# g1n0st/drake

Measured on AMD Instinct MI355X. Metric: mpm_substeps_per_sec_1M_particles, higher is better.
Workload: dtype f32

## Files before the change

### drake_amd/csrc/mpm_device.h

```cpp
#pragma once
#include <hip/hip_runtime.h>
#include <stdint.h>

#include "mpm_math.h"

namespace mpm {

constexpr int FREE_ZONE = 2;
constexpr int TILE_W = 4 + 2 * FREE_ZONE + 2;
constexpr int TILE_N = TILE_W * TILE_W * TILE_W;

constexpr unsigned ERR_DRIFT = 1u;
constexpr unsigned ERR_CAPACITY = 2u;
constexpr unsigned ERR_DOMAIN = 4u;
constexpr unsigned ERR_RANGE = 8u;
constexpr unsigned ERR_HALO = 16u;
constexpr unsigned ERR_SLABS = 32u;

constexpr unsigned VF_MARK = 0x7FB0A5C3u;
constexpr unsigned VF_CHUNK = 32;
__host__ __device__ inline size_t vf_entry(unsigned k, unsigned j) {
    return (size_t)(k / VF_CHUNK) * (8u * VF_CHUNK) + j * VF_CHUNK + (k % VF_CHUNK);
}
struct PSet {
    float4* q[4];
    int* pid;
    float4* fq[4];
    float* f8;
    float* c8;
};

MPM_DEV void unpack_C(const float4& q1, const float4& q2, const float4& q3, float* C) {
    C[0] = q2.x; C[1] = q2.y; C[2] = q2.z; C[3] = q2.w;
    C[4] = q3.x; C[5] = q3.y; C[6] = q3.z; C[7] = q3.w;
    C[8] = q1.w;
}

struct Ctl {
    int cur;
    int need_rebuild;
    unsigned error;
    unsigned skipped;
    int skip_this;
    unsigned watch_hit;
    unsigned n_home;
    unsigned n_active;
    unsigned n_items;
    unsigned rebuilds;
    unsigned ticket;
    int nfa, nva;
    int add_f, add_v;
    int nfa_new, nva_new;
    unsigned n_items_wanted;
    float quiet_time;
    float time_since_resort;
    float mig_quiet;
};

struct Dist {
    int on;
    int rank, world;
    int own_lo, own_hi;
    int nbr_lo, nbr_hi;
    int has_left, has_right;
    float ghost_w;
    float vert_w;
    float hyst;
    int zone_cells;
    float mig_delta;
    float mig_reach;
    unsigned* mig_min;
    unsigned char* prev;
};

MPM_DEV float dist_xi(float x, float dxinv) { return x * dxinv - .5f; }
MPM_DEV bool dist_in_my_band(const Dist& d, int bx, float xi, bool face, float extra = 0.f) {
    const float w = (face ? d.ghost_w : d.vert_w) + extra;
    return (d.has_left && bx < d.own_lo && xi >= (float)d.own_lo - w) || (d.has_right && bx >= d.own_hi && xi < (float)d.own_hi + w);
}
MPM_DEV int dist_in_neighbour_bands(const Dist& d, float xi, bool face, int old = 0) {
    const float w = face ? d.ghost_w : d.vert_w;
    const float wl = w + ((old & 1) ? d.hyst : 0.f), wr = w + ((old & 2) ? d.hyst : 0.f);
    return ((d.has_left && xi < (float)d.own_lo + wl) ? 1 : 0) | ((d.has_right && xi >= (float)d.own_hi - wr) ? 2 : 0);
}

struct DP {
    int Np, Nf, Nv;
    int NpG, NfG;
    int bits;
    int nb;
    unsigned nblocks, ncells;
    unsigned capH, capA, capI;
    unsigned capS;
    int item_groups;
    int item_groups_small;
    int item_small_below;
    int dbg;
    float dx, dxinv, Dinv;
    unsigned q_stride, f_stride;
    int gated;
    unsigned watch_base;
    int lean_resort;
    int lean_g2p;
    int fem_fast;
    float anticip;
    double fix_m, fix_p, unfix_m, unfix_p;
    Material M;
    Ctl* ctl;
    unsigned long long* dbgbuf;
    PSet set[2];
    int4* fg[2];
    int4* vg[2][2];
    float3* ta;
    float3* G3;
    float* VF;
    float* f[3];
    const int* idx_orig[3];
    const int* adj_off;
    const int* adj_fc;
    int* imap;
    uint32_t* pkey;
    uint32_t* prank;
    uint32_t* src_of;
    int* dst_of;
    unsigned* tickets;
    uint32_t* halo_hdr[2];
    int halo_cls, halo_nz, halo_zlo[2], halo_zhi[2];
    int halo_pn, halo_plo[2], halo_phi[2], halo_pshift[2];
    unsigned halo_pcap;
    uint32_t* halo_pbuf[2];
    uint32_t* halo_pcnt[2];
    int* cellcnt[2];
    int* blkcnt[2];
    int* blkstart[2];
    int* lut_home;
    int* lut_act;
    unsigned* home_bits;
    uint32_t* home_block;
    int4* home_range;
    int* home_nbr_act;
    int4* item_desc;
    uint32_t* item_order;
    int4* item_flat;
    int4* item_rng;
    uint32_t* item_pos;
    int2* home_items;
    int* act_nbr_items;
    int* home_ngroups;
    int4* home_groups;
    uint32_t* act_block;
    int* act_nbr_home;
    float4* slab;
    uint32_t* slab_mask;
    float4* gv;
    float4* gvs;
    const float4* dm_orig;
    Dist dist;
};

MPM_DEV int active_slot(const DP& p, int idx, int nf_in) { return idx < nf_in ? idx : p.Nf + (idx - nf_in); }

#ifndef MPM_DIAG
#define MPM_DIAG 0
#endif
MPM_DEV int diag_flags(const DP& p) { return MPM_DIAG ? p.dbg : 0; }

MPM_DEV void pack_F(const float* F, float4& r0, float4& r1, float& r2) {
    r0 = make_float4(F[2], F[5], F[8], F[0]);
    r1 = make_float4(F[1], F[3], F[4], F[6]);
    r2 = F[7];
}
MPM_DEV void unpack_F(const float4& r0, const float4& r1, float r2, float* F) {
    F[2] = r0.x; F[5] = r0.y; F[8] = r0.z; F[0] = r0.w;
    F[1] = r1.x; F[3] = r1.y; F[4] = r1.z; F[6] = r1.w;
    F[7] = r2;
}
// ... 41 lines not shown
```

### drake_amd/csrc/mpm_engine.hip

```cpp
#include <hip/hip_runtime.h>

#include <algorithm>
#include <chrono>
#include <cmath>
#include <cstdio>
#include <cstdlib>
#include <cstring>
#include <fstream>
#include <functional>
#include <mutex>
#include <numeric>
#include <string>
#include <thread>
#include <vector>

#include "../../include/mpm_hip.h"
#include "mpm_host.h"
#include "mpm_io.h"
#include "mpm_debug_tables.h"
#include "mpm_contact.h"
#include "mpm_chain.h"
#include "mpm_feedback.h"
#include "mpm_dist.h"
#include "mpm_cloth_host.h"
#include "mpm_bodies_host.h"
#include "mpm_dist_host.h"
#include "mpm_chain_host.h"

static std::mutex g_live_mutex;
static std::vector<mpm_engine*> g_live;

extern "C" {

const char* mpm_last_error(void) { return g_last_error.c_str(); }

int mpm_default_material(mpm_material_t* m) try {
    REQUIRE(m, "null material");
    m->youngs_modulus = 400000.f;
    m->poisson_ratio = .3f;
    m->density = 2000.f;
    m->gamma = 0.f;
    m->K = 100000.f;
    m->V = .8f;
    m->c_F = 0.f;
    m->sdf_friction = .3f;
    m->gravity = -9.8f;
    m->epsv = 1e-3f;
    m->gravity_axis = 2;
    m->wall_cells = 3;
    return 0;
} MPM_CATCH_ALL

int mpm_create(int domain_bits, const mpm_material_t* material, int device, mpm_handle_t* out) try {
    REQUIRE(out, "null handle pointer");
    REQUIRE(domain_bits >= 4 && domain_bits <= 8, "domain_bits must be in [4,8] (16^3 .. 256^3 cells)");
    int ndev = 0;
    if (hipGetDeviceCount(&ndev) != hipSuccess || ndev <= 0)
        return fail(MPM_ERR_NO_DEVICE, "no HIP device visible: the engine has no CPU fallback");
    REQUIRE(device >= 0 && device < ndev, "device ordinal out of range");
    mpm_engine* e = new mpm_engine();
    e->device = device;
    e->bits = domain_bits;
    if (material) e->mat = *material; else mpm_default_material(&e->mat);
    if (e->mat.gravity_axis < 0 || e->mat.gravity_axis > 2) {
        delete e;
        return fail(MPM_ERR_INVALID, "gravity_axis must be 0, 1 or 2");
    }
    hipError_t err = hipSetDevice(device);
    if (err == hipSuccess) err = hipStreamCreateWithFlags(&e->own_stream, hipStreamNonBlocking);
    if (err != hipSuccess) {
        delete e;
        return fail(MPM_ERR_HIP, std::string("mpm_create: ") + hipGetErrorString(err));
    }
    e->stream = e->own_stream;
    if (getenv("MPM_RESORT_EVERY")) e->check_every = std::max(1, atoi(getenv("MPM_RESORT_EVERY")));
    if (getenv("MPM_DEFER_PHASES")) e->defer_phases = atoi(getenv("MPM_DEFER_PHASES")) != 0;
    if (getenv("MPM_QUIET_FACTOR")) e->quiet_factor = std::min(1.f, std::max(0.f, (float)atof(getenv("MPM_QUIET_FACTOR"))));
    {
        std::lock_guard<std::mutex> lock(g_live_mutex);
        g_live.push_back(e);
    }
    *out = e;
    return 0;
} MPM_CATCH_ALL

static int add_cloth(mpm_engine* e, const float* pos, const float* vel, size_t n_verts, const int32_t* indices,
                     size_t n_faces, const mpm_cloth_material_t* m) {
    REQUIRE(e, "null handle");
    REQUIRE(!e->finalized, "AddQRCloth after Finalize");
    REQUIRE(pos && vel && (indices || n_faces == 0), "null input array");
    for (size_t i = 0; i < n_faces * 3; ++i)
        REQUIRE(indices[i] >= 0 && (size_t)indices[i] < n_verts, "triangle index out of range");
    REQUIRE(!(e->multi_mat || m) || e->cloths.size() < MAX_CLOTH_MATERIALS,
            "more than 256 cloths in a multi-material engine (mpm_add_qr_cloth_with_material)");
    mpm_engine::Cloth c{e->nv, n_verts, e->nf, n_faces, {}};
    c.m = m ? *m : engine_cloth_material(e);
    e->cloths.push_back(c);
    if (m) e->multi_mat = true;
    for (size_t i = 0; i < n_faces * 3; ++i) e->h_idx.push_back(indices[i] + (int)e->nv);
    e->h_pos.insert(e->h_pos.end(), pos, pos + 3 * n_verts);
    e->h_vel.insert(e->h_vel.end(), vel, vel + 3 * n_verts);
    e->nv += n_verts;
    e->nf += n_faces;
    e->np = e->nv + e->nf;
    return 0;
}

int mpm_add_qr_cloth(mpm_handle_t e, const float* pos, const float* vel, size_t n_verts, const int32_t* indices,
                     size_t n_faces) try {
    return add_cloth(e, pos, vel, n_verts, indices, n_faces, nullptr);
} MPM_CATCH_ALL

int mpm_add_qr_cloth_with_material(mpm_handle_t e, const float* pos, const float* vel, size_t n_verts,
                                   const int32_t* indices, size_t n_faces, const mpm_cloth_material_t* m) try {
    REQUIRE(e, "null handle");
    const mpm_cloth_material_t c = m ? *m : engine_cloth_material(e);
    REQUIRE(std::isfinite(c.youngs_modulus) && std::isfinite(c.poisson_ratio) && std::isfinite(c.density) &&
                std::isfinite(c.gamma) && std::isfinite(c.K) && std::isfinite(c.c_F),
            "cloth material: a field is not finite");
    REQUIRE(c.youngs_modulus > 0.f, "cloth material: youngs_modulus must be > 0");
    REQUIRE(c.poisson_ratio >= 0.f && c.poisson_ratio < .5f, "cloth material: poisson_ratio must be in [0, 0.5)");
    REQUIRE(c.density > 0.f, "cloth material: density must be > 0");
    REQUIRE(c.gamma >= 0.f && c.K >= 0.f && c.c_F >= 0.f, "cloth material: gamma, K and c_F must be >= 0");
    return add_cloth(e, pos, vel, n_verts, indices, n_faces, &c);
} MPM_CATCH_ALL

int mpm_cloth_count(mpm_handle_t e, size_t* n_out) try {
    REQUIRE(e && n_out, "null argument");
    *n_out = e->cloths.size();
    return 0;
} MPM_CATCH_ALL

int mpm_get_cloth_info(mpm_handle_t e, size_t cloth, size_t* first_vertex, size_t* n_verts, size_t* first_face,
                       size_t* n_faces, mpm_cloth_material_t* m) try {
    REQUIRE(e, "null handle");
    REQUIRE(cloth < e->cloths.size(), "cloth index out of range");
    const mpm_engine::Cloth& c = e->cloths[cloth];
    if (first_vertex) *first_vertex = c.first_vertex;
    if (n_verts) *n_verts = c.n_verts;
    if (first_face) *first_face = c.first_face;
    if (n_faces) *n_faces = c.n_faces;
    if (m) *m = c.m;
    return 0;
} MPM_CATCH_ALL

static void launch_rebuild(mpm_engine* e, DP p, bool lean, float dt) {
    if (dt > 0.f) e->last_dt = dt;
    p.anticip = e->anticipation();
    p.lean_resort = lean && !p.dist.on;
    e->checks_launched += 1;
    TraceRange tr("mpm:RebuildMapping (conditional re-sort)");
    hipLaunchKernelGGL(k_rb_count, dim3(std::min(e->g_np, e->g_rb)), dim3(256), 0, e->stream, p);
    hipLaunchKernelGGL(k_rb_tables, dim3(33), dim3(1024), 0, e->stream, p);
    hipLaunchKernelGGL(k_rb_scatter, dim3(std::min(e->g_np, e->g_rb)), dim3(256), 0, e->stream, p);
    if (e->deterministic) hipLaunchKernelGGL(k_rb_canon, dim3(512), dim3(256), 0, e->stream, p);
    hipLaunchKernelGGL(k_rb_finish, dim3((std::min(e->g_np, e->g_rb) + 7u) & ~7u), dim3(256), 0, e->stream, p);
}

static void launch_fem_faces(mpm_engine* e, const DP& p, float dt) {
    TraceRange tr("mpm:CalcFemStateAndForce (faces)");
    if (!e->nf) return;
    const dim3 g((e->g_nf + 7u) & ~7u), b(256);
    if (e->multi_mat) {
        const ClothMat* t = e->d_cloth_mat;
        if (e->fast_math) hipLaunchKernelGGL(k_fem_mat<1>, g, b, 0, e->stream, p, dt, t);
        else hipLaunchKernelGGL(k_fem_mat<0>, g, b, 0, e->stream, p, dt, t);
    } else if (e->fast_math) hipLaunchKernelGGL(k_fem<1>, g, b, 0, e->stream, p, dt);
    else hipLaunchKernelGGL(k_fem<0>, g, b, 0, e->stream, p, dt);
    if (e->damp.membrane()) hipLaunchKernelGGL(k_damp, g, b, 0, e->stream, p, e->damp.args);
}
static void launch_fem_vertices(mpm_engine* e, const DP& p, float dt) {
    TraceRange tr("mpm:CalcFemStateAndForce (vertex forces)");
    if (e->nv) hipLaunchKernelGGL(k_vforce, dim3((e->g_nv + 7u) & ~7u), dim3(256), 0, e->stream, p);
    if (e->bend.on()) hipLaunchKernelGGL(k_bend, rows_grid(e->bend.args.n_rows), dim3(256), 0, e->stream, p, e->bend.args);
    if (e->bend.on() && e->damp.bending())
        hipLaunchKernelGGL(k_bend_damp, rows_grid(e->bend.args.n_rows), dim3(256), 0, e->stream, p, e->bend.args,
                           (const float*)e->damp.d_beta_vertex);
    if (e->links.on()) hipLaunchKernelGGL(k_link, rows_grid(e->links.args.n_rows), dim3(256), 0, e->stream, p, e->links.args);
    if (e->pressure.on()) {
        const mpm_engine::Pressure& ps = e->pressure;
        if (ps.gas()) {
            PressureVolumeArgs va = ps.vol;
            va.ranges = ps.d_ranges_gas;
            va.only_gas = 1;
            hipLaunchKernelGGL(k_pressure_volume, dim3((unsigned)ps.n_gas_chunks), dim3(256), 0, e->stream, p, va, 0);
            hipLaunchKernelGGL(k_pressure_gauge, dim3((unsigned)e->cloths.size()), dim3(64), 0, e->stream, p, va);
        }
        hipLaunchKernelGGL(k_pressure, rows_grid(ps.args.n_rows), dim3(256), 0, e->stream, p, ps.args);
    }
    if (e->shell.on()) {
        hipLaunchKernelGGL(k_hinge, rows_grid(e->shell.hinge.n), dim3(256), 0, e->stream, p, e->shell.hinge);
        hipLaunchKernelGGL(k_hinge_gather, rows_grid(e->shell.args.n_rows), dim3(256), 0, e->stream, p, e->shell.args);
    }
    if (e->anchors.on()) {
        const AnchorArgs a = anchors_posed(e);
        const AnchorAcc acc{e->cb.body_acc, (int)e->cb.n_bodies, p.fix_p};
        hipLaunchKernelGGL(k_anchor, rows_grid(a.n_rows), dim3(256), 0, e->stream, p, a, acc, dt);
    }
}
static void launch_fem(mpm_engine* e, const DP& p, float dt) {
    e->last_dt = dt;
    launch_fem_faces(e, p, dt);
    launch_fem_vertices(e, p, dt);
}
static void launch_p2g(mpm_engine* e, const DP& p, float dt, int forces = 0) {
    TraceRange tr(forces ? "mpm:ParticleToGrid (+ vertex forces)" : "mpm:ParticleToGrid");
    const dim3 g(e->g_tile), b(P2G_THREADS);
    const bool exact = e->deterministic || e->p2g_fixed_point;
#define MPM_P2G_LAUNCH(F)                                                                          \
    do {                                                                                           \
        if (exact) hipLaunchKernelGGL((k_p2g<F, 1>), g, b, 0, e->stream, p, dt);                   \
        else hipLaunchKernelGGL((k_p2g<F, 0>), g, b, 0, e->stream, p, dt);                         \
    } while (0)
#define MPM_P2G_LAUNCH_FIELDS(F)                                                                                      \
    do {                                                                                                              \
        const ForceFieldTable* t = e->d_force_fields;                                                                 \
        if (exact) hipLaunchKernelGGL((k_p2g<F, 1, 1, ForceFieldTable>), g, b, 0, e->stream, p, dt, t);        \
        else hipLaunchKernelGGL((k_p2g<F, 0, 1, ForceFieldTable>), g, b, 0, e->stream, p, dt, t);              \
    } while (0)
    if (!e->force_fields.empty()) {
        if (forces == 1) MPM_P2G_LAUNCH_FIELDS(1);
        else MPM_P2G_LAUNCH_FIELDS(0);
    } else if (forces == 1) MPM_P2G_LAUNCH(1);
    else MPM_P2G_LAUNCH(0);
#undef MPM_P2G_LAUNCH_FIELDS
#undef MPM_P2G_LAUNCH
}
static int fused_forces(const mpm_engine* e) {
    return e->max_valence <= 8 && !e->bend.on() && !e->links.on() && !e->pressure.on() && !e->shell.on() && !e->anchors.on() ? 1 : 0;
}
static void launch_pins(mpm_engine* e, const DP& p, float dt) {
    TraceRange tr("mpm:Pins");
    const mpm_engine::PinState& ps = e->pin;
    PinArgs a{ps.d_pins, (int)ps.set.size(), ps.d_mot, (int)ps.motion_body.size(), e->cb.body_acc, (int)e->cb.n_bodies,
              p.fix_p, ps.d_ticket};
    const unsigned groups = (unsigned)std::max<size_t>(1, std::min<size_t>((ps.set.size() + 255) / 256, 1024));
    hipLaunchKernelGGL(k_pin, dim3(groups), dim3(256), 0, e->stream, p, a, dt);
}
static void launch_g2p(mpm_engine* e, const DP& p, float dt) {
    TraceRange tr("mpm:GridToParticle");
    hipLaunchKernelGGL(k_g2p, dim3(std::min(768u, p.capI)), dim3(G2P_THREADS), 0, e->stream, p, dt);
    if ((!e->pin.set.empty() || e->anchors.on()) && p.halo_cls < 0) launch_pins(e, p, dt);
}
static void launch_grid(mpm_engine* e, const DP& p, const GridColliders& gc) {
    TraceRange tr("mpm:UpdateGrid");
    if (gc.n < 0) {
        const dim3 g(e->g_grid), b(256);
        const GridBodyTable* t = e->d_grid_bodies;
        long long* acc = e->cb.body_acc;
        const int nb = (int)e->cb.n_bodies;
        switch (e->grid_bodies_kinds) {
            case 0: hipLaunchKernelGGL(k_grid_bodies<0>, g, b, 0, e->stream, p, t, acc, nb); break;
            case 1: hipLaunchKernelGGL(k_grid_bodies<1>, g, b, 0, e->stream, p, t, acc, nb); break;
            case 2: hipLaunchKernelGGL(k_grid_bodies<2>, g, b, 0, e->stream, p, t, acc, nb); break;
            default: hipLaunchKernelGGL(k_grid_bodies<3>, g, b, 0, e->stream, p, t, acc, nb); break;
        }
        return;
    }
    hipLaunchKernelGGL(k_grid<1>, dim3(e->g_grid), dim3(256), 0, e->stream, p, gc);
}

using PhaseMark = std::function<void(int)>;
enum class Resort { None, Lean, Full, Held };
static void enqueue_substep_front(mpm_engine* e, const DP& p, float dt, Resort resort, const PhaseMark& mark = {}) {
    if (resort != Resort::None) launch_rebuild(e, p, resort == Resort::Lean, resort == Resort::Held ? 0.f : dt);
    e->last_dt = dt;
    if (mark) mark(MPM_PHASE_REBUILD);
    launch_fem_faces(e, p, dt);
    if (mark) mark(MPM_PHASE_FEM);
    const int forces = fused_forces(e);
    if (!forces) launch_fem_vertices(e, p, dt);
    if (mark) mark(MPM_PHASE_VFORCE);
    launch_p2g(e, p, dt, forces);
    if (mark) mark(MPM_PHASE_P2G);
}
enum class GridForm { Fused, Gather, FromSums };
static void enqueue_substep_rest(mpm_engine* e, GridForm form, const DP& pg, const GridColliders& gc, const DP* p2, float dt,
                                 const PhaseMark& mark = {}) {
    const dim3 g(e->g_grid), b(256);
    switch (form) {
        case GridForm::Fused: launch_grid(e, pg, gc); break;
        case GridForm::Gather: hipLaunchKernelGGL(k_grid<0>, g, b, 0, e->stream, pg, GridColliders{}); break;
        case GridForm::FromSums: hipLaunchKernelGGL(k_grid<2>, g, b, 0, e->stream, pg, gc); break;
    }
    if (mark) mark(MPM_PHASE_GRID);
    if (!p2) return;
    launch_g2p(e, *p2, dt);
    if (mark) mark(MPM_PHASE_G2P);
}

static int set_fixed_point_scales(mpm_engine* e) {
    DP& p = e->dp;
    const size_t slots = (size_t)p.Np;
    std::vector<float> q0(slots * 4);
    HIP_TRY(hipStreamSynchronize(e->stream));
    Ctl c;
    D2H(e, &c, p.ctl, sizeof(Ctl));
    D2H(e, q0.data(), p.set[c.cur & 1].q[0], slots * 16);
    double mass = 0;
    for (size_t i = 0; i < slots; ++i) mass += std::fabs((double)q0[i * 4 + 3]) * p.M.density;
    if (!(mass > 0) || !std::isfinite(mass)) mass = 1.0;
    const int k = 61 - (int)std::ceil(std::log2(mass));
    p.fix_m = std::ldexp(1.0, k);
    p.fix_p = std::ldexp(1.0, k - 14);
    p.unfix_m = 1.0 / p.fix_m;
    p.unfix_p = 1.0 / p.fix_p;
    return 0;
}

int mpm_finalize(mpm_handle_t e) try {
    REQUIRE(e, "null handle");
    REQUIRE(!e->finalized, "Finalize called twice");
    REQUIRE(e->np > 0, "no particles: call mpm_add_qr_cloth first");
    if (int rc = use(e)) return rc;
    const size_t np = e->np, nf = e->nf, nv = e->nv;
    REQUIRE(np < (size_t)1 << 30, "too many particles");
    DP& p = e->dp;
    p.Np = (int)np; p.Nf = (int)nf; p.Nv = (int)nv;
    p.NpG = (int)np; p.NfG = (int)nf;
    p.bits = e->bits;
    p.dbg = getenv("MPM_DBG") ? atoi(getenv("MPM_DBG")) : 0;
    p.nb = 1 << (e->bits - 2);
    p.ncells = 1u << (3 * e->bits);
    p.nblocks = p.ncells >> 6;
    p.capH = (unsigned)std::min<size_t>(p.nblocks, np);
    p.capA = (unsigned)std::min<size_t>(p.nblocks, (size_t)27 * p.capH);
    p.halo_cls = -1;
    p.fem_fast = e->fast_math ? 1 : 0;
    p.item_groups = getenv("MPM_ITEM_GROUPS") ? std::max(1, atoi(getenv("MPM_ITEM_GROUPS"))) : 48;
    p.item_groups_small = getenv("MPM_ITEM_GROUPS_SMALL") ? std::max(1, atoi(getenv("MPM_ITEM_GROUPS_SMALL"))) : 16;
    p.item_small_below = getenv("MPM_ITEM_SMALL_BELOW") ? atoi(getenv("MPM_ITEM_SMALL_BELOW")) : 6500;
    p.capI = p.capH + (unsigned)(np / (64 * (size_t)std::min(p.item_groups, p.item_groups_small))) + 16u;
    p.capS = (unsigned)std::min<size_t>(p.capI, std::max<size_t>(4096, np / 256 + 1024 + np / (64 * (size_t)p.item_groups)));
    if (getenv("MPM_SLAB_CAPACITY")) p.capS = (unsigned)std::min<size_t>(p.capI, std::max(1, atoi(getenv("MPM_SLAB_CAPACITY"))));
    p.dxinv = (float)(1 << e->bits);
    p.dx = 1.f / p.dxinv;
    p.Dinv = 4.f * p.dxinv * p.dxinv;
    const mpm_material_t& m = e->mat;
    lame(m.youngs_modulus, m.poisson_ratio, &p.M.mu, &p.M.lambda);
    p.M.density = m.density; p.M.gamma = m.gamma; p.M.K = m.K; p.M.V = m.V; p.M.cF = m.c_F;
    if (e->multi_mat) p.M.density = 1.f;
    p.M.sdf_friction = m.sdf_friction; p.M.gravity = m.gravity; p.M.epsv = m.epsv;
    p.M.gravity_axis = m.gravity_axis; p.M.wall = m.wall_cells;

    int rc = 0;
    p.q_stride = (unsigned)((np + 63) & ~(size_t)63);
    p.f_stride = (unsigned)((np + 63) & ~(size_t)63);
#define ALLOC(ptr, n, zero)                         \
    if ((rc = e->dalloc(&(ptr), (n), (zero)))) return rc
    ALLOC(p.ctl, 1, true);
    ALLOC(p.dbgbuf, 16, true);
    for (int s = 0; s < 2; ++s) {
        PSet& S = p.set[s];
        {
            float4* base = nullptr;
            ALLOC(base, 4 * (size_t)p.q_stride, true);
            for (int d = 0; d < 4; ++d) S.q[d] = base + (size_t)d * p.q_stride;
        }
        for (int d = 0; d < 4; ++d) ALLOC(S.fq[d], nf, true);
        ALLOC(S.f8, nf, true);
        ALLOC(S.c8, nf, true);
        ALLOC(S.pid, np, true);
    }
    ALLOC(p.ta, std::max<size_t>(nf, 1), true);
    ALLOC(p.G3, 3 * nf, true);
    ALLOC(p.VF, 3 * vf_entry((unsigned)nv + VF_CHUNK, 0), true);
    {
        float* base = nullptr;
        ALLOC(base, 3 * (size_t)p.f_stride, true);
        for (int d = 0; d < 3; ++d) p.f[d] = base + (size_t)d * p.f_stride;
    }
    int* idx_orig[3];
    int *adj_off, *adj_fc;
    for (int d = 0; d < 3; ++d) { ALLOC(idx_orig[d], nf, false); p.idx_orig[d] = idx_orig[d]; }
    ALLOC(adj_off, nv + 1, false);
    ALLOC(adj_fc, 3 * nf, false);
    p.adj_off = adj_off; p.adj_fc = adj_fc;
// ... 1910 lines not shown
```

### drake_amd/csrc/mpm_step.h

```cpp
#pragma once
#include "mpm_device.h"
#include "mpm_fields.h"
#include "mpm_zone_buffer.h"

namespace mpm {

MPM_DEV bool gated_out(const DP& p) {
    return ((p.gated & 1) && p.ctl->need_rebuild) || ((p.gated & 2) && (p.ctl->error & ERR_SLABS)) ||
           ((p.gated & 4) && (int)(p.ctl->watch_hit - p.watch_base) >= 0);
}

template <int FM>
__global__ __launch_bounds__(256) void k_fem(DP p, float dt) {
#define MPM_FEM_MATERIAL_SETUP
#define MPM_FEM_M p.M
#define MPM_FEM_VOLW p.dist.on ? S.q[0][i].w : f2.w
#include "mpm_fem_face.inc"
#undef MPM_FEM_MATERIAL_SETUP
#undef MPM_FEM_M
#undef MPM_FEM_VOLW
}

struct ClothMat {
    float mu, lambda, gamma, K, cF, rho, pad0, pad1;
};
constexpr int FACE_CLOTH_SHIFT = 12;
MPM_DEV Material cloth_material(const Material& engine, const ClothMat* mats, const float4& f3) {
    const ClothMat t = mats[(unsigned)__float_as_int(f3.x) >> FACE_CLOTH_SHIFT];
    Material m = engine;
    m.mu = t.mu; m.lambda = t.lambda; m.gamma = t.gamma; m.K = t.K; m.cF = t.cF; m.density = t.rho;
    return m;
}

template <int FM>
__global__ __launch_bounds__(256) void k_fem_mat(DP p, float dt, const ClothMat* mats) {
#define MPM_FEM_MATERIAL_SETUP const Material M = cloth_material(p.M, mats, f3);
#define MPM_FEM_M M
#define MPM_FEM_VOLW f2.w * M.density
#include "mpm_fem_face.inc"
#undef MPM_FEM_MATERIAL_SETUP
#undef MPM_FEM_M
#undef MPM_FEM_VOLW
}

MPM_DEV bool vertex_force_vf(const DP& p, int k, float& f0, float& f1, float& f2) {
    const float* e0 = p.VF + vf_entry((unsigned)k, 0) * 3;
    float3 g[8];
#pragma unroll
    for (int j = 0; j < 8; ++j) g[j] = *reinterpret_cast<const float3*>(e0 + (size_t)j * VF_CHUNK * 3);
    f0 = f1 = f2 = 0.f;
#pragma unroll
    for (int j = 0; j < 8; ++j) {
        f0 += -g[j].x;
        f1 += -g[j].y;
        f2 += -g[j].z;
    }
    return __float_as_uint(g[0].x) != VF_MARK;
}

MPM_DEV void vertex_force_csr(const DP& p, const PSet& S, int k, float& f0, float& f1, float& f2) {
    const int s = p.Nf + k;
    f0 = f1 = f2 = 0.f;
    const int vo = S.pid[s] - p.NfG;
    for (int e = p.adj_off[vo]; e < p.adj_off[vo + 1]; ++e) {
        const int fc = p.adj_fc[e];
        const int fs = p.imap[fc >> 2];
        const float3 g = fs >= 0 ? p.G3[(size_t)fs * 3 + (fc & 3)]
                                 : make_float3(S.q[0][s].w > 0.f ? __int_as_float(0x7FC00000) : 0.f, 0.f, 0.f);
        f0 += -g.x;
        f1 += -g.y;
        f2 += -g.z;
    }
}

MPM_DEV void vertex_force_value(const DP& p, const PSet& S, int k, float& f0, float& f1, float& f2) {
    if (!vertex_force_vf(p, k, f0, f1, f2)) vertex_force_csr(p, S, k, f0, f1, f2);
}
MPM_DEV void vertex_force(const DP& p, const PSet& S, int k) {
    float f0, f1, f2;
    vertex_force_value(p, S, k, f0, f1, f2);
    const int s = p.Nf + k;
    p.f[0][s] = f0;
    p.f[1][s] = f1;
    p.f[2][s] = f2;
}

__global__ __launch_bounds__(256) void k_vforce(DP p) {
    if (gated_out(p)) return;
    const unsigned nva = (unsigned)p.ctl->nva;
    const unsigned chunk = xcd_chunk_active(blockIdx.x, nva);
    const int k = (int)(chunk * 256 + threadIdx.x);
    if (chunk == 0xFFFFFFFFu || k >= (int)nva) return;
    vertex_force(p, p.set[p.ctl->cur], k);
}

typedef float f32x4 __attribute__((ext_vector_type(4)));
typedef float f32x2 __attribute__((ext_vector_type(2)));

constexpr int STG = 23, STG_PXY = 8, STG_FZ = 17, STG_ROWS = 67;
MPM_DEV int stg_col(int c) { return c < 8 ? c : c + 10; }

MPM_DEV void lds_add_fixed(long long* a, float q, unsigned& worst) {
    const float aq = fabsf(q);
    const float h = floorf(aq * 0x1p-32f);
    const unsigned lo = (unsigned)rintf(fmaf(-h, 0x1p32f, aq));
    const unsigned long long mag = ((unsigned long long)(unsigned)h << 32) | lo;
    const unsigned long long fx = q < 0.f ? 0ull - mag : mag;
    __hip_atomic_fetch_add(reinterpret_cast<unsigned long long*>(a), fx, __ATOMIC_RELAXED,
                           __HIP_MEMORY_SCOPE_WORKGROUP);
    worst = max(worst, __float_as_uint(aq));
}

MPM_DEV void bspline_coeff(int a, bool on, float& c0, float& c1, float& c2) {
    c0 = a == 0 ? 1.125f : (a == 1 ? -.25f : .125f);
    c1 = a == 0 ? -1.5f : (a == 1 ? 2.f : -.5f);
    c2 = a == 1 ? -1.f : .5f;
    if (!on) c0 = c1 = c2 = 0.f;
}

struct Stencil {
    int rx, ry, rz;
    float fx[3];
    float wx[3], wy[3], wz[3];
    unsigned out_bits;
};

MPM_DEV Stencil make_stencil(const DP& p, float x, float y, float z, int ox, int oy, int oz) {
    Stencil s;
    const uint32_t hi = (uint32_t)((1 << p.bits) - 3);
    const uint32_t bx = min(base_cell(x, p.dxinv), hi), by = min(base_cell(y, p.dxinv), hi),
                   bz = min(base_cell(z, p.dxinv), hi);
    s.fx[0] = x * p.dxinv - (float)bx;
    s.fx[1] = y * p.dxinv - (float)by;
    s.fx[2] = z * p.dxinv - (float)bz;
    bspline3(s.fx[0], s.wx);
    bspline3(s.fx[1], s.wy);
    bspline3(s.fx[2], s.wz);
    int rx = (int)bx - ox, ry = (int)by - oy, rz = (int)bz - oz;
    const int hi_h = TILE_W - 3;
    static_assert(((TILE_W - 3) & (TILE_W - 2)) == 0, "rx | ry | rz <= hi_h is only equivalent to all three in range for hi_h = 2^k - 1");
    s.out_bits = (unsigned)(rx | ry | rz);
    rx = min(max(rx, 0), hi_h);
    ry = min(max(ry, 0), hi_h);
    rz = min(max(rz, 0), hi_h);
    s.rx = rx; s.ry = ry; s.rz = rz;
    return s;
}

MPM_DEV unsigned tile_reach_mask(int rx, int ry, int rz) {
    static_assert(FREE_ZONE == 2, "the packed tables below are for a free zone of 2 cells");
    const int ix = rx >> 1, iy = ry >> 1, iz = rz >> 1;
    const unsigned long long Z = 0x926D924DBull, Y = 0xE07E0703Full;
    const unsigned m9 = (unsigned)((Z >> (9 * iz)) & (Y >> (9 * iy))) & 0x1FFu;
    const unsigned rep = m9 * 0x40201u;
    const int lo = (ix + 1) >> 1, hi = (ix >> 1) + 1;
    const unsigned xexp = ((1u << (9 * (hi + 1))) - 1u) ^ ((1u << (9 * lo)) - 1u);
    return rep & xexp;
}

constexpr int P2G_WAVES = 8, P2G_THREADS = 64 * P2G_WAVES;
MPM_DEV f32x4 p2g_mfma(float y, float w, f32x4 acc) { return __builtin_amdgcn_mfma_f32_16x16x4f32(y, w, acc, 0, 0, 0); }
MPM_DEV const ForceFieldTable* p2g_field_table(const ForceFieldTable* t) { return t; }
template <int FORCES, int EXACT, int FIELDS = 0, typename... TABLE>
__global__ __launch_bounds__(P2G_THREADS) __attribute__((amdgpu_waves_per_eu(P2G_WAVES / 2, P2G_WAVES / 2))) void k_p2g(DP p, float dt, const TABLE* __restrict__... table) {
    static_assert(sizeof...(TABLE) == FIELDS, "the table is the argument of the FIELDS = 1 instances only");
    if (gated_out(p)) return;
    if (blockIdx.x == 0 && threadIdx.x < 2 && p.halo_hdr[threadIdx.x]) p.halo_hdr[threadIdx.x][0] = 0u;
    __shared__ long long tile[TILE_N * 4];
    __shared__ __attribute__((aligned(16))) float stage_all[P2G_WAVES][STG_ROWS * STG];
    __shared__ unsigned s_mask;
    static_assert(sizeof(long long) * TILE_N * 4 + sizeof(float) * P2G_WAVES * STG_ROWS * STG + 4 <= 81920,
                  "two workgroups per CU need <= 80 KB of LDS each");
    Ctl* ctl = p.ctl;
    const PSet& S = p.set[ctl->cur];
    const int tid = threadIdx.x, lane = tid & 63, wv = tid >> 6;
    const float gdt = p.M.gravity * dt;
    const float sdt = -dt * p.Dinv;
    float* stage = stage_all[wv];

    const int j16 = lane & 15, g4 = lane >> 4;
    const int node[2] = {j16 < 15 ? j16 : -1, j16 >= 3 && j16 < 15 ? j16 + 12 : -1};
    float cz0, cz1, cz2;
    bspline_coeff(j16 % 3, true, cz0, cz1, cz2);
    const int ycol = j16 < 13 ? stg_col(j16) : 0;
    const int xycol = STG_PXY + j16 / 3;
    float fac[2][4];
    int delta[2];
#pragma unroll
    for (int t = 0; t < 2; ++t) {
        const int n = node[t];
        const int ni = n / 9, nj = (n / 3) % 3, nk = n % 3;
#pragma unroll
        for (int r = 0; r < 4; ++r) {
            fac[t][r] = n < 0 ? 0.f : (r == 0 ? 1.f : (float)(r == 1 ? ni : (r == 2 ? nj : nk)));
            if (g4 == 3 && r != 0) fac[t][r] = 0.f;
        }
        delta[t] = n >= 0 ? ((ni * TILE_W + nj) * TILE_W + nk) * 4 + g4 : -1;
    }
    {
        const float fscale = EXACT ? (float)(g4 == 3 ? p.fix_m : p.fix_p) : 1.f;
#pragma unroll
        for (int t = 0; t < 2; ++t)
#pragma unroll
            for (int r = 0; r < 4; ++r) fac[t][r] *= fscale;
    }
    const unsigned reach_of_lane = tile_reach_mask(2 * (lane >> 4), 2 * ((lane >> 2) & 3), 2 * (lane & 3));
    for (int k = lane; k < STG_ROWS * STG; k += 64) stage[k] = 0.f;

    const unsigned n_items = ctl->n_items;
    for (unsigned q = blockIdx.x; q < n_items; q += gridDim.x) {
        __syncthreads();
        const int4 fa = p.item_flat[2 * q], fb = p.item_flat[2 * q + 1];
        const unsigned item = (unsigned)fa.x;
        const unsigned long long tb0 = (diag_flags(p) & 4) ? __builtin_readcyclecounter() : 0ull;
        for (int n = tid; n < TILE_N * 4; n += P2G_THREADS) tile[n] = 0;
        if (tid == 0) s_mask = 0;
        int bx, by, bz;
        block_coords((uint32_t)fa.z, bx, by, bz);
        const int ox = bx * 4 - FREE_ZONE, oy = by * 4 - FREE_ZONE, oz = bz * 4 - FREE_ZONE;
        const int4 rg = make_int4(fb.x, fb.y, fb.z, 0);
        const int nfb = rg.y - rg.x;
        const int ngroups = fa.w;
        const int4* groups = p.home_groups + fb.w;
        struct Raw {
            float x[3], v[3], vol, C[9];
            float ta[3], tb[3], frc[3];
            bool act, is_face;
        };
        auto force_of = [&](unsigned ii, float* f) {
            const float* fbase = p.f[0] + ii;
#pragma unroll
            for (int d = 0; d < 3; ++d) f[d] = fbase[(size_t)d * p.f_stride];
        };
        auto desc_of = [&](int g) { return groups[min(g, ngroups - 1)]; };
        int4 gd_next = make_int4(0, 0, 0, 0);
        auto load_raw = [&](int4 gr) {
            Raw r;
            const int gf = gr.y - gr.x, gn = gf + (gr.w - gr.z);
            r.act = lane < gn;
            r.is_face = lane < gf;
            const unsigned any_slot = (unsigned)(nfb ? rg.x : rg.z);
            const unsigned ii = r.act ? (unsigned)(r.is_face ? gr.x + lane : gr.z + (lane - gf)) : any_slot;
            const float4* qb = S.q[0] + ii;
            const float4 q0 = qb[0], q1 = qb[p.q_stride], q2 = qb[2 * (size_t)p.q_stride], q3 = qb[3 * (size_t)p.q_stride];
            r.x[0] = q0.x; r.x[1] = q0.y; r.x[2] = q0.z; r.vol = q0.w;
            r.v[0] = q1.x; r.v[1] = q1.y; r.v[2] = q1.z;
            unpack_C(q1, q2, q3, r.C);
            {
                const unsigned fi = r.is_face ? ii : (unsigned)(nfb ? rg.x : 0), vi = r.is_face ? any_slot : ii;
                const float3 a = p.ta[fi];
                const float3 b = *reinterpret_cast<const float3*>(&S.fq[0][fi]);
                r.ta[0] = a.x; r.ta[1] = a.y; r.ta[2] = a.z; r.tb[0] = b.x; r.tb[1] = b.y; r.tb[2] = b.z;
                const bool vert = r.act && !r.is_face;
                if (FORCES == 1) {
                    vertex_force_vf(p, vert ? (int)ii - p.Nf : 0, r.frc[0], r.frc[1], r.frc[2]);
                } else {
                    force_of(vi, r.frc);
                }
                if (FORCES != 0 && vert && !p.lean_g2p) {
                    p.f[0][ii] = r.frc[0]; p.f[1][ii] = r.frc[1]; p.f[2][ii] = r.frc[2];
                }
            }
            return r;
        };
        Raw cur;
        __syncthreads();
        unsigned mymask = 0;
        bool halo_bad = false;
        unsigned out_worst = 0, fix_worst = 0;
        if (wv < ngroups) gd_next = desc_of(wv);
        const bool prof = (diag_flags(p) & 4) != 0 && wv == 0;
        unsigned long long tq[3] = {0, 0, 0}, pc[8] = {0, 0, 0, 0, 0, 0, 0, 0};
        if (prof && lane == 0) atomicAdd(&p.dbgbuf[14], (unsigned long long)__builtin_readcyclecounter() - tb0);
        for (int g = wv; g < ngroups; g += P2G_WAVES) {
            if (prof) tq[0] = __builtin_readcyclecounter();
            cur = load_raw(gd_next);
            gd_next = desc_of(g + P2G_WAVES);
            const bool act = cur.act, is_face = cur.is_face;
            const Stencil st = make_stencil(p, cur.x[0], cur.x[1], cur.x[2], ox, oy, oz);
            const bool own = cur.vol > 0.f;
            const float m = own ? cur.vol * p.M.density : 0.f;
            float Y[16];
            {
                float B[9];
                float fext[3] = {0.f, 0.f, 0.f};
#pragma unroll
                for (int r = 0; r < 9; ++r) B[r] = cur.C[r] * m;
                if (is_face) {
#pragma unroll
                    for (int r = 0; r < 3; ++r)
#pragma unroll
                        for (int c = 0; c < 3; ++c) B[r * 3 + c] = fmaf(sdt, cur.ta[r] * cur.tb[c], B[r * 3 + c]);
                } else {
#pragma unroll
                    for (int r = 0; r < 3; ++r) fext[r] = cur.frc[r] * dt;
                }
                if constexpr (FIELDS != 0) {
                    const ForceFieldTable* ft = p2g_field_table(table...);
                    float a[3];
                    force_field_acceleration(ft->f, ft->n, cur.x, cur.v, cur.tb, is_face, a);
#pragma unroll
                    for (int r = 0; r < 3; ++r) fext[r] = fmaf(m, a[r] * dt, fext[r]);
                }
#pragma unroll
                for (int r = 0; r < 3; ++r) {
                    float qq = r == p.M.gravity_axis ? fmaf(cur.v[r], m, m * gdt) : cur.v[r] * m;
                    qq += fext[r];
                    const float dot = fmaf(B[r * 3 + 2], st.fx[2], fmaf(B[r * 3], st.fx[0], B[r * 3 + 1] * st.fx[1]));
                    qq = fmaf(-p.dx, dot, qq);
                    Y[r * 4 + 0] = qq;
                    Y[r * 4 + 1] = B[r * 3 + 0] * p.dx;
                    Y[r * 4 + 2] = B[r * 3 + 1] * p.dx;
                    Y[r * 4 + 3] = B[r * 3 + 2] * p.dx;
                }
                Y[12] = m; Y[13] = 0.f; Y[14] = 0.f; Y[15] = 0.f;
                if (p.dist.on && !own) {
#pragma unroll
                    for (int k = 0; k < 12; ++k) Y[k] = 0.f;
                }
            }
            out_worst = max(out_worst, act ? st.out_bits : 0u);
            if (p.dist.on && act && own) {
                const int gx = ox + st.rx;
                halo_bad |= gx < p.dist.own_lo - p.dist.zone_cells || gx + 2 >= p.dist.own_hi + p.dist.zone_cells;
            }
            if (diag_flags(p) & 2) {
                float acc = 0.f;
#pragma unroll
                for (int k = 0; k < 16; ++k) acc += Y[k];
                if (acc == 1.2345e30f) tile[0] = (long long)acc;
                continue;
            }
            const int key = (st.rx * 8 + st.ry) * 8 + st.rz;
            const unsigned long long actmask = __ballot(act);
            int pos = 0;
            {
                unsigned long long todo = actmask;
                int base = 0;
                while (todo) {
                    const int lk = __builtin_amdgcn_readlane(key, __builtin_ctzll(todo));
                    const bool mine = key == lk;
                    const unsigned long long same = __ballot(mine) & todo;
                    const int rank = (int)__builtin_amdgcn_mbcnt_hi((unsigned)(same >> 32), __builtin_amdgcn_mbcnt_lo((unsigned)same, (unsigned)base));
                    if (mine) pos = rank;
                    base += (int)__popcll(same);
                    todo &= ~same;
                }
            }
            if (act) {
                float px[3], py[3];
#pragma unroll
                for (int a = 0; a < 3; ++a) {
                    float c0, c1, c2;
                    bspline_coeff(a, true, c0, c1, c2);
                    px[a] = fmaf(fmaf(c2, st.fx[0], c1), st.fx[0], c0);
                    py[a] = fmaf(fmaf(c2, st.fx[1], c1), st.fx[1], c0);
                }
                float* sp = stage + pos * STG;
#pragma unroll
                for (int c = 0; c < 13; ++c) sp[stg_col(c)] = Y[c];
#pragma unroll
                for (int a = 0; a < 9; ++a) sp[STG_PXY + a] = px[a / 3] * py[a % 3];
                sp[STG_FZ] = st.fx[2];
            }
            __builtin_amdgcn_fence(__ATOMIC_RELEASE, "wavefront");
            __builtin_amdgcn_wave_barrier();
            __builtin_amdgcn_fence(__ATOMIC_ACQUIRE, "wavefront");
            if (diag_flags(p) & 1) continue;
            unsigned long long todo = actmask;
            int s0 = 0;
            float ny, nfz;
            f32x2 nxy;
            const float *ry, *rxy, *rz;
            auto load_ops = [&](int off) {
                ny = ry[off]; nxy = f32x2{rxy[off], rxy[off + 4]}; nfz = rz[off];
            };
            auto cell_rows = [&](int s) {
                const float* row = stage + (s + g4) * STG;
                ry = row + ycol; rxy = row + xycol; rz = row + STG_FZ;
                load_ops(0);
            };
            cell_rows(0);
            if (prof) tq[1] = __builtin_readcyclecounter();
            __builtin_amdgcn_s_setprio(2);
            while (todo) {
                const int ckey = __builtin_amdgcn_readlane(key, __builtin_ctzll(todo));
                const unsigned long long same = __ballot(key == ckey) & todo;
                todo &= ~same;
                const int s1 = s0 + __builtin_popcount((unsigned)same) + __builtin_popcount((unsigned)(same >> 32));
                const int nsteps = (s1 - s0 + 3) >> 2;
                f32x4 acc0 = {0.f, 0.f, 0.f, 0.f}, acc1 = {0.f, 0.f, 0.f, 0.f};
                if (prof) { pc[4] += 1; pc[5] += (unsigned)nsteps; tq[2] = __builtin_readcyclecounter(); }
                auto step = [&](int k, bool first_step, bool last_step) {
                    const float pz = fmaf(fmaf(cz2, nfz, cz1), nfz, cz0);
                    const f32x2 w01 = nxy * f32x2{pz, pz};
                    float y = ny;
                    if (last_step && !(g4 < s1 - s0 - 4 * k)) y = 0.f;
                    if (first_step) {
                        const f32x4 zero = {0.f, 0.f, 0.f, 0.f};
                        acc0 = p2g_mfma(y, w01.x, zero);
                        acc1 = p2g_mfma(y, w01.y, zero);
                    } else {
                        acc0 = p2g_mfma(y, w01.x, acc0);
                        acc1 = p2g_mfma(y, w01.y, acc1);
                    }
                    if (!last_step) load_ops(4 * (k + 1) * STG);
                };
                if (nsteps == 1) {
                    step(0, true, true);
                } else {
                    step(0, true, false);
#define MPM_P2G_MIDDLE(k) if (nsteps - 1 == k) goto last_step; step(k, false, false);
                    MPM_P2G_MIDDLE(1) MPM_P2G_MIDDLE(2) MPM_P2G_MIDDLE(3) MPM_P2G_MIDDLE(4) MPM_P2G_MIDDLE(5)
                    MPM_P2G_MIDDLE(6) MPM_P2G_MIDDLE(7) MPM_P2G_MIDDLE(8) MPM_P2G_MIDDLE(9) MPM_P2G_MIDDLE(10)
                    MPM_P2G_MIDDLE(11) MPM_P2G_MIDDLE(12) MPM_P2G_MIDDLE(13) MPM_P2G_MIDDLE(14)
#undef MPM_P2G_MIDDLE
                last_step:
                    step(nsteps - 1, false, true);
                }
                cell_rows(min(s1, 63));
                if (prof) { asm volatile("" :: "v"(acc0), "v"(acc1)); const unsigned long long tm = __builtin_readcyclecounter(); pc[2] += tm - tq[2]; tq[2] = tm; }
                s0 = s1;
                const int crx = ckey >> 6, cry = (ckey >> 3) & 7, crz = ckey & 7;
                mymask |= (unsigned)__builtin_amdgcn_readlane((int)reach_of_lane, ((ckey >> 3) & 0x30) | ((ckey >> 2) & 0xC) | ((ckey >> 1) & 3));
                long long* tb = tile + ((crx * TILE_W + cry) * TILE_W + crz) * 4;
#pragma unroll
                for (int t = 0; t < 2; ++t) {
                    const f32x4 a = t ? acc1 : acc0;
                    float val;
                    {
#pragma clang fp contract(off)
                        const float x0 = a[0] * fac[t][0], x1 = a[1] * fac[t][1], x2 = a[2] * fac[t][2], x3 = a[3] * fac[t][3];
                        val = (x0 + x1) + (x2 + x3);
                    }
                    if (delta[t] >= 0 && !(diag_flags(p) & 16)) {
                        if (EXACT) lds_add_fixed(tb + delta[t], val, fix_worst);
                        else __hip_atomic_fetch_add(reinterpret_cast<double*>(tb + delta[t]), (double)val, __ATOMIC_RELAXED, __HIP_MEMORY_SCOPE_WORKGROUP);
                    }
                }
                if (prof) pc[3] += __builtin_readcyclecounter() - tq[2];
            }
            if (prof) {
                const unsigned long long te = __builtin_readcyclecounter();
                pc[0] += tq[1] - tq[0];
                pc[1] += te - tq[1];
                pc[6] += 1;
            }
            __builtin_amdgcn_s_setprio(0);
            __builtin_amdgcn_fence(__ATOMIC_RELEASE, "wavefront");
            __builtin_amdgcn_wave_barrier();
        }
        if (prof) pc[7] = __builtin_readcyclecounter() - tb0;
        if (prof && lane == 0)
            for (int q = 0; q < 8; ++q) atomicAdd(&p.dbgbuf[q], pc[q]);
        if (mymask && lane == 0) atomicOr(&s_mask, mymask);
        if (__ballot(out_worst > (unsigned)(TILE_W - 3)) && lane == 0) atomicOr(&ctl->error, ERR_DRIFT);
        if (EXACT && __ballot(fix_worst >= __float_as_uint(0x1p62f)) && lane == 0) atomicOr(&ctl->error, ERR_RANGE);
        if (p.dist.on && __ballot(halo_bad) && lane == 0) atomicOr(&ctl->error, ERR_HALO);
        __syncthreads();
        if (prof && lane == 0) atomicAdd(&p.dbgbuf[15], (unsigned long long)__builtin_readcyclecounter() - tb0 - pc[7]);
        float4* out = p.slab + (size_t)item * TILE_N;
        bool not_finite = false;
        for (int n = tid; n < TILE_N; n += P2G_THREADS) {
            const long long* q = tile + n * 4;
            float4 o;
            if (EXACT) {
                o = make_float4((float)((double)q[0] * p.unfix_p), (float)((double)q[1] * p.unfix_p),
                                (float)((double)q[2] * p.unfix_p), (float)((double)q[3] * p.unfix_m));
            } else {
                const double* d = reinterpret_cast<const double*>(q);
                o = make_float4((float)d[0], (float)d[1], (float)d[2], (float)d[3]);
                not_finite |= !(fabsf(o.x) + fabsf(o.y) + fabsf(o.z) + fabsf(o.w) < __int_as_float(0x7F800000));
            }
            out[n] = o;
        }
        if (!EXACT && __ballot(not_finite) && lane == 0) atomicOr(&ctl->error, ERR_RANGE);
        if (tid == 0) p.slab_mask[item] = s_mask;
        if ((diag_flags(p) & 4) && tid == 0) {
            atomicAdd(&p.dbgbuf[12], (unsigned long long)__builtin_readcyclecounter() - tb0);
            atomicAdd(&p.dbgbuf[13], 1ull);
        }
    }
}

struct GridCollider {
    int shape;
    int mode;
    float p[3], n[3], radius, v[3], friction;
};
constexpr int MAX_GRID_COLLIDERS = 16;
struct GridColliders {
    int n;
    GridCollider c[MAX_GRID_COLLIDERS];
};

constexpr int GRID_LIST = 160;
MPM_DEV int __reduce_max_sync_i32(int v) {
#pragma unroll
    for (int d = 32; d >= 1; d >>= 1) v = max(v, __shfl_xor(v, d));
    return v;
}

template <int MODE>
__global__ __launch_bounds__(256) void k_grid(DP p, GridColliders gc) {
#define MPM_GRID_BODIES 0
#include "mpm_grid_update.inc"
#undef MPM_GRID_BODIES
}

constexpr int G2P_THREADS = 512, G2P_WAVES = 4;
constexpr int LOAD_TILE_NQ = (TILE_N + G2P_THREADS - 1) / G2P_THREADS;
MPM_DEV void load_tile(const DP& p, unsigned h, float4* tile, const float4* field, int nthreads, unsigned long long* stamps = nullptr) {
    const int* nbr = p.home_nbr_act + (size_t)h * 27;
    constexpr int NQ = LOAD_TILE_NQ;
    int a[NQ], cell[NQ];
#pragma unroll
    for (int q = 0; q < NQ; ++q) {
        const int n = min((int)threadIdx.x + q * nthreads, TILE_N - 1);
        const int tx = n / (TILE_W * TILE_W), ty = (n / TILE_W) % TILE_W, tz = n % TILE_W;
        const int qx = tx - FREE_ZONE + 4, qy = ty - FREE_ZONE + 4, qz = tz - FREE_ZONE + 4;
        a[q] = nbr[(qx >> 2) * 9 + (qy >> 2) * 3 + (qz >> 2)];
        cell[q] = ((qx & 3) << 4) + ((qy & 3) << 2) + (qz & 3);
    }
    if (MPM_DIAG && stamps) { asm volatile("s_waitcnt vmcnt(0)" ::: "memory"); stamps[0] = __builtin_readcyclecounter(); }
    float4 v[NQ];
#pragma unroll
    for (int q = 0; q < NQ; ++q) v[q] = field[(size_t)max(a[q], 0) * 64 + cell[q]];
    if (MPM_DIAG && stamps) { asm volatile("s_waitcnt vmcnt(0)" ::: "memory"); stamps[1] = __builtin_readcyclecounter(); }
#pragma unroll
    for (int q = 0; q < NQ; ++q) {
        const int n = (int)threadIdx.x + q * nthreads;
        if (n < TILE_N) tile[n] = a[q] >= 0 ? v[q] : make_float4(0.f, 0.f, 0.f, 0.f);
    }
}

MPM_DEV int g2p_particle(const DP& p, const PSet& S, const float4* tile, unsigned i, float x, float y, float z,
                            float vol, int ox, int oy, int oz, float dt) {
    const Stencil st = make_stencil(p, x, y, z, ox, oy, oz);
    int bits = 0;
    if (p.dist.on && vol < 0.f) {
        const int gx = ox + st.rx;
        if (gx < p.dist.own_lo - p.dist.zone_cells || gx + 2 >= p.dist.own_hi + p.dist.zone_cells) bits = 2;
    }
    float nv[3] = {0.f, 0.f, 0.f}, nC[9] = {0.f, 0.f, 0.f, 0.f, 0.f, 0.f, 0.f, 0.f, 0.f};
    const float4* base = tile + ((st.rx * TILE_W + st.ry) * TILE_W + st.rz);
    const float ez[3] = {st.wz[0] * (0.f - st.fx[2]), st.wz[1] * (1.f - st.fx[2]), st.wz[2] * (2.f - st.fx[2])};
    const float ey[3] = {st.wy[0] * (0.f - st.fx[1]), st.wy[1] * (1.f - st.fx[1]), st.wy[2] * (2.f - st.fx[1])};
    const f32x2 W0 = {st.wz[0], ez[0]}, W1 = {st.wz[1], ez[1]}, W2 = {st.wz[2], ez[2]};
    const f32x2 zero2 = {0.f, 0.f};
#pragma unroll
    for (int a = 0; a < 3; ++a) {
        f32x2 BB[3] = {zero2, zero2, zero2};
        float By[3] = {0.f, 0.f, 0.f};
#pragma unroll
        for (int b = 0; b < 3; ++b) {
            const float4* row = base + (a * TILE_W + b) * TILE_W;
            const float4 g0 = row[0], g1 = row[1], g2 = row[2];
            const float wb = st.wy[b], eb = ey[b];
            const f32x2 wb2 = {wb, wb};
            const float c0[3] = {g0.x, g0.y, g0.z}, c1[3] = {g1.x, g1.y, g1.z}, c2[3] = {g2.x, g2.y, g2.z};
#pragma unroll
            for (int r = 0; r < 3; ++r) {
                f32x2 AA;
                if (r == 2) {
                    const f32x2 z0 = {g0.z, g0.w}, z1 = {g1.z, g1.w}, z2 = {g2.z, g2.w};
                    asm("v_pk_mul_f32 %0, %1, %2 op_sel_hi:[1,0]\n\ts_nop 0\n\t"
                        "v_pk_fma_f32 %0, %3, %4, %0 op_sel_hi:[1,0,1]\n\ts_nop 0\n\t"
                        "v_pk_fma_f32 %0, %5, %6, %0 op_sel_hi:[1,0,1]"
                        : "=&v"(AA) : "v"(W0), "v"(z0), "v"(W1), "v"(z1), "v"(W2), "v"(z2));
                } else {
                    const f32x2 s0 = {c0[r], c0[r]}, s1 = {c1[r], c1[r]}, s2 = {c2[r], c2[r]};
                    AA = __builtin_elementwise_fma(W2, s2, __builtin_elementwise_fma(W1, s1, W0 * s0));
                }
                BB[r] = __builtin_elementwise_fma(wb2, AA, BB[r]);
                By[r] = fmaf(eb, AA.x, By[r]);
            }
        }
        const float wa = st.wx[a];
        const float ea = wa * ((float)a - st.fx[0]);
        const f32x2 wa2 = {wa, wa};
#pragma unroll
        for (int r = 0; r < 3; ++r) {
            f32x2 vc = {nv[r], nC[r * 3 + 2]};
            vc = __builtin_elementwise_fma(wa2, BB[r], vc);
            nv[r] = vc.x;
            nC[r * 3 + 2] = vc.y;
// ... 147 lines not shown
```

Measured before the change: 10030.

## Specialize vertex-force gather to six planes when mesh valence allows

Adds a PLANES template parameter to the vertex-force gather and the P2G kernel, so meshes with a maximum valence of six or less read only six of the eight per-vertex force planes and skip the CSR fallback check. This cuts global memory loads in k_vforce and in the fused P2G force path. It also rewrites the P2G accumulation reduction to use FMAs and, in the non-exact path, drops one multiply (assuming fac[t][0] is one). The FMA change alters rounding, and the dropped multiply depends on that factor really being one.

```diff
diff --git a/drake_amd/csrc/mpm_device.h b/drake_amd/csrc/mpm_device.h
--- a/drake_amd/csrc/mpm_device.h
+++ b/drake_amd/csrc/mpm_device.h
@@ -22,6 +22,8 @@
 __host__ __device__ inline size_t vf_entry(unsigned k, unsigned j) {
     return (size_t)(k / VF_CHUNK) * (8u * VF_CHUNK) + j * VF_CHUNK + (k % VF_CHUNK);
 }
+constexpr int VF_PLANES_REGULAR = 6, VF_PLANES_ALL = 8;
+__host__ __device__ inline int vf_planes_of(int max_valence) { return max_valence <= VF_PLANES_REGULAR ? VF_PLANES_REGULAR : VF_PLANES_ALL; }
 struct PSet {
     float4* q[4];
     int* pid;
diff --git a/drake_amd/csrc/mpm_engine.hip b/drake_amd/csrc/mpm_engine.hip
--- a/drake_amd/csrc/mpm_engine.hip
+++ b/drake_amd/csrc/mpm_engine.hip
@@ -171,7 +171,11 @@
 }
 static void launch_fem_vertices(mpm_engine* e, const DP& p, float dt) {
     TraceRange tr("mpm:CalcFemStateAndForce (vertex forces)");
-    if (e->nv) hipLaunchKernelGGL(k_vforce, dim3((e->g_nv + 7u) & ~7u), dim3(256), 0, e->stream, p);
+    if (e->nv) {
+        const dim3 g((e->g_nv + 7u) & ~7u), b(256);
+        if (vf_planes_of(e->max_valence) == VF_PLANES_REGULAR) hipLaunchKernelGGL(k_vforce<VF_PLANES_REGULAR>, g, b, 0, e->stream, p);
+        else hipLaunchKernelGGL(k_vforce<VF_PLANES_ALL>, g, b, 0, e->stream, p);
+    }
     if (e->bend.on()) hipLaunchKernelGGL(k_bend, rows_grid(e->bend.args.n_rows), dim3(256), 0, e->stream, p, e->bend.args);
     if (e->bend.on() && e->damp.bending())
         hipLaunchKernelGGL(k_bend_damp, rows_grid(e->bend.args.n_rows), dim3(256), 0, e->stream, p, e->bend.args,
@@ -207,22 +211,25 @@
     TraceRange tr(forces ? "mpm:ParticleToGrid (+ vertex forces)" : "mpm:ParticleToGrid");
     const dim3 g(e->g_tile), b(P2G_THREADS);
     const bool exact = e->deterministic || e->p2g_fixed_point;
-#define MPM_P2G_LAUNCH(F)                                                                          \
+#define MPM_P2G_LAUNCH(F, V)                                                                       \
     do {                                                                                           \
-        if (exact) hipLaunchKernelGGL((k_p2g<F, 1>), g, b, 0, e->stream, p, dt);                   \
-        else hipLaunchKernelGGL((k_p2g<F, 0>), g, b, 0, e->stream, p, dt);                         \
+        if (exact) hipLaunchKernelGGL((k_p2g<F, 1, 0, V>), g, b, 0, e->stream, p, dt);             \
+        else hipLaunchKernelGGL((k_p2g<F, 0, 0, V>), g, b, 0, e->stream, p, dt);                   \
     } while (0)
-#define MPM_P2G_LAUNCH_FIELDS(F)                                                                                      \
+#define MPM_P2G_LAUNCH_FIELDS(F, V)                                                                                   \
     do {                                                                                                              \
         const ForceFieldTable* t = e->d_force_fields;                                                                 \
-        if (exact) hipLaunchKernelGGL((k_p2g<F, 1, 1, ForceFieldTable>), g, b, 0, e->stream, p, dt, t);        \
-        else hipLaunchKernelGGL((k_p2g<F, 0, 1, ForceFieldTable>), g, b, 0, e->stream, p, dt, t);              \
+        if (exact) hipLaunchKernelGGL((k_p2g<F, 1, 1, V, ForceFieldTable>), g, b, 0, e->stream, p, dt, t);     \
+        else hipLaunchKernelGGL((k_p2g<F, 0, 1, V, ForceFieldTable>), g, b, 0, e->stream, p, dt, t);           \
     } while (0)
+    const bool regular = vf_planes_of(e->max_valence) == VF_PLANES_REGULAR;
     if (!e->force_fields.empty()) {
-        if (forces == 1) MPM_P2G_LAUNCH_FIELDS(1);
-        else MPM_P2G_LAUNCH_FIELDS(0);
-    } else if (forces == 1) MPM_P2G_LAUNCH(1);
-    else MPM_P2G_LAUNCH(0);
+        if (forces == 1 && regular) MPM_P2G_LAUNCH_FIELDS(1, VF_PLANES_REGULAR);
+        else if (forces == 1) MPM_P2G_LAUNCH_FIELDS(1, VF_PLANES_ALL);
+        else MPM_P2G_LAUNCH_FIELDS(0, VF_PLANES_ALL);
+    } else if (forces == 1 && regular) MPM_P2G_LAUNCH(1, VF_PLANES_REGULAR);
+    else if (forces == 1) MPM_P2G_LAUNCH(1, VF_PLANES_ALL);
+    else MPM_P2G_LAUNCH(0, VF_PLANES_ALL);
 #undef MPM_P2G_LAUNCH_FIELDS
 #undef MPM_P2G_LAUNCH
 }
diff --git a/drake_amd/csrc/mpm_step.h b/drake_amd/csrc/mpm_step.h
--- a/drake_amd/csrc/mpm_step.h
+++ b/drake_amd/csrc/mpm_step.h
@@ -43,19 +43,21 @@
 #undef MPM_FEM_VOLW
 }
 
+template <int PLANES>
 MPM_DEV bool vertex_force_vf(const DP& p, int k, float& f0, float& f1, float& f2) {
+    static_assert(PLANES == VF_PLANES_REGULAR || PLANES == VF_PLANES_ALL, "the two instances the launches choose between");
     const float* e0 = p.VF + vf_entry((unsigned)k, 0) * 3;
-    float3 g[8];
-#pragma unroll
-    for (int j = 0; j < 8; ++j) g[j] = *reinterpret_cast<const float3*>(e0 + (size_t)j * VF_CHUNK * 3);
+    float3 g[PLANES];
+#pragma unroll
+    for (int j = 0; j < PLANES; ++j) g[j] = *reinterpret_cast<const float3*>(e0 + (size_t)j * VF_CHUNK * 3);
     f0 = f1 = f2 = 0.f;
 #pragma unroll
-    for (int j = 0; j < 8; ++j) {
+    for (int j = 0; j < PLANES; ++j) {
         f0 += -g[j].x;
         f1 += -g[j].y;
         f2 += -g[j].z;
     }
-    return __float_as_uint(g[0].x) != VF_MARK;
+    return PLANES < VF_PLANES_ALL || __float_as_uint(g[0].x) != VF_MARK;
 }
 
 MPM_DEV void vertex_force_csr(const DP& p, const PSet& S, int k, float& f0, float& f1, float& f2) {
@@ -73,25 +75,28 @@
     }
 }
 
+template <int PLANES>
 MPM_DEV void vertex_force_value(const DP& p, const PSet& S, int k, float& f0, float& f1, float& f2) {
-    if (!vertex_force_vf(p, k, f0, f1, f2)) vertex_force_csr(p, S, k, f0, f1, f2);
-}
+    if (!vertex_force_vf<PLANES>(p, k, f0, f1, f2)) vertex_force_csr(p, S, k, f0, f1, f2);
+}
+template <int PLANES>
 MPM_DEV void vertex_force(const DP& p, const PSet& S, int k) {
     float f0, f1, f2;
-    vertex_force_value(p, S, k, f0, f1, f2);
+    vertex_force_value<PLANES>(p, S, k, f0, f1, f2);
     const int s = p.Nf + k;
     p.f[0][s] = f0;
     p.f[1][s] = f1;
     p.f[2][s] = f2;
 }
 
+template <int PLANES>
 __global__ __launch_bounds__(256) void k_vforce(DP p) {
     if (gated_out(p)) return;
     const unsigned nva = (unsigned)p.ctl->nva;
     const unsigned chunk = xcd_chunk_active(blockIdx.x, nva);
     const int k = (int)(chunk * 256 + threadIdx.x);
     if (chunk == 0xFFFFFFFFu || k >= (int)nva) return;
-    vertex_force(p, p.set[p.ctl->cur], k);
+    vertex_force<PLANES>(p, p.set[p.ctl->cur], k);
 }
 
 typedef float f32x4 __attribute__((ext_vector_type(4)));
@@ -161,7 +166,7 @@
 constexpr int P2G_WAVES = 8, P2G_THREADS = 64 * P2G_WAVES;
 MPM_DEV f32x4 p2g_mfma(float y, float w, f32x4 acc) { return __builtin_amdgcn_mfma_f32_16x16x4f32(y, w, acc, 0, 0, 0); }
 MPM_DEV const ForceFieldTable* p2g_field_table(const ForceFieldTable* t) { return t; }
-template <int FORCES, int EXACT, int FIELDS = 0, typename... TABLE>
+template <int FORCES, int EXACT, int FIELDS = 0, int PLANES = VF_PLANES_ALL, typename... TABLE>
 __global__ __launch_bounds__(P2G_THREADS) __attribute__((amdgpu_waves_per_eu(P2G_WAVES / 2, P2G_WAVES / 2))) void k_p2g(DP p, float dt, const TABLE* __restrict__... table) {
     static_assert(sizeof...(TABLE) == FIELDS, "the table is the argument of the FIELDS = 1 instances only");
     if (gated_out(p)) return;
@@ -253,7 +258,7 @@
                 r.ta[0] = a.x; r.ta[1] = a.y; r.ta[2] = a.z; r.tb[0] = b.x; r.tb[1] = b.y; r.tb[2] = b.z;
                 const bool vert = r.act && !r.is_face;
                 if (FORCES == 1) {
-                    vertex_force_vf(p, vert ? (int)ii - p.Nf : 0, r.frc[0], r.frc[1], r.frc[2]);
+                    vertex_force_vf<PLANES>(p, vert ? (int)ii - p.Nf : 0, r.frc[0], r.frc[1], r.frc[2]);
                 } else {
                     force_of(vi, r.frc);
                 }
@@ -430,8 +435,8 @@
                     float val;
                     {
 #pragma clang fp contract(off)
-                        const float x0 = a[0] * fac[t][0], x1 = a[1] * fac[t][1], x2 = a[2] * fac[t][2], x3 = a[3] * fac[t][3];
-                        val = (x0 + x1) + (x2 + x3);
+                        const float x0 = EXACT ? a[0] * fac[t][0] : a[0], x2 = a[2] * fac[t][2];
+                        val = fmaf(a[1], fac[t][1], x0) + fmaf(a[3], fac[t][3], x2);
                     }
                     if (delta[t] >= 0 && !(diag_flags(p) & 16)) {
                         if (EXACT) lds_add_fixed(tb + delta[t], val, fix_worst);
```

Result: faster. 10150, median of 6 (+1.2%).
